# neggles/neurosis

Hardware: AMD Instinct MI355X
Metric: train images/sec (node) SDXL 1024^2 (higher is better)
Workload: dtype bf16

## Files before the change

include/neurosis_hip.h:

```cpp
#ifndef NEUROSIS_HIP_H
#define NEUROSIS_HIP_H

#ifdef __cplusplus
extern "C" {
#endif

const char* nk_last_error(void);
int nk_abi_version(void);

int nk_linear_fwd(const void* x, const void* w, const float* bias, const void* residual, void* y,
                  int M, int N, int K, long ldx, long ldw, long ldr, long ldy, float alpha, void* stream);
int nk_linear_dgrad(const void* dy, const void* w, const void* dx_add, void* dx, int M, int N, int K,
                    long lddy, long ldw, long ldadd, long lddx, void* stream);
long nk_linear_fwd_geglu_ok(int M, int I, int K);
int nk_linear_fwd_geglu(const void* x, const void* w, const float* bias, void* u, void* h, int M, int I, int K, long ldx, long ldw, long ldu,
                        long ldh, void* stream);
int nk_linear_dgrad_geglu(const void* dy, const void* w, const void* u, void* du, int M, int N, int I, long lddy, long ldw, long ldu,
                          long lddu, void* stream);
int nk_linear_fwd_geglu_s(const void* x, const void* w, const float* bias, void* s, void* h, int M, int I, int K, long ldx, long ldw, long lds,
                          long ldh, void* stream);
int nk_linear_dgrad_geglu_s(const void* dy, const void* w, const void* s, void* du, int M, int N, int I, long lddy, long ldw, long lds,
                            long lddu, void* stream);
int nk_linear_wgrad(const void* dy, const void* x, float* dw, int M, int N, int K, long lddy, long ldx,
                    long lddw, int accumulate, void* stream);
int nk_linear_wgrad_bias(const void* dy, const void* x, float* dw, float* dbias, int M, int N, int K, long lddy, long ldx, long lddw,
                         int accumulate, void* stream);

int nk_gemm_sk_status(void);

int nk_health_status(void);
int nk_health_clear(void);
int nk_health_export(int* dst, void* stream);
int nk_health_import(const int* src, void* stream);
int nk_debug_raise_health(void* stream);
int nk_debug_stamp(unsigned long long* dst, void* stream);
int nk_debug_launch_log(int mode);
long nk_debug_launch_names(char* buf, long cap);

int nk_colsum_batched(const void* dy, float* out, float* ws, long M, int N, long ld, int nbatch, int accumulate, void* stream);

int nk_linear_fwd_batched(const void* const* x, const void* const* w, void* const* y, int count, int M, int N, int K,
                          long ldx, long ldw, long ldy, void* stream);

int nk_linear_wgrad_batched(const void* const* dy, const void* const* x, float* const* dw, float* const* dbias, int count, int M, int N,
                            int K, long lddy, long ldx, long lddw, int accumulate, void* stream);

typedef struct NkConvDesc {
  int N, H, W, Cin;
  int Cout, KH, KW;
  int stride;
  int pad_t, pad_l;
  int Ho, Wo;
  int upsample;
} NkConvDesc;
int nk_conv2d_fwd(const NkConvDesc* d, const void* x, const void* w, const float* bias, const void* rowvec,
                  const void* residual, void* y, void* stream);
long nk_conv2d_stats_tiles(const NkConvDesc* d, int stats_groups);
int nk_conv2d_fwd_stats(const NkConvDesc* d, const void* x, const void* w, const float* bias, const void* rowvec, const void* residual,
                        void* y, float* stats_part, int stats_groups, void* stream);
int nk_conv3x3_few_channels_fwd(const void* x, const void* w, const float* bias, void* y, int N, int H, int W, int Cout, int cin_real,
                                void* stream);
int nk_conv_weight_flip(const void* w, void* wt, int Cout, int Cin, int taps, void* stream);
long nk_conv2d_dgrad_flipped_ok(const NkConvDesc* d);
int nk_conv2d_dgrad_flipped(const NkConvDesc* d, const void* dy, const void* wt, void* dx, void* stream);
int nk_conv2d_dgrad(const NkConvDesc* d, const void* dy, const void* w, void* dx, void* stream);
int nk_conv2d_wgrad(const NkConvDesc* d, const void* dy, const void* x, float* dw, int accumulate, void* stream);
int nk_conv2d_wgrad_bias(const NkConvDesc* d, const void* dy, const void* x, float* dw, float* dbias, int accumulate, void* stream);

typedef struct NkAttnDesc {
  int B, H, Lq, Lk, D;
  long sq, sk, sv, so;
  long bq, bk, bv, bo;
  long sdq, sdk, sdv, sdo;
  long bdq, bdk, bdv, bdo;
  float scale;
  int causal;
} NkAttnDesc;
int nk_attention_fwd(const NkAttnDesc* d, const void* q, const void* k, const void* v, void* o, float* lse,
                     void* stream);
long nk_attention_bwd_ws_floats(const NkAttnDesc* d);
int nk_attention_bwd(const NkAttnDesc* d, const void* q, const void* k, const void* v, const void* o,
// ... 166 lines not shown
```

neurosis_amd/csrc/conv_halo.h:

```cpp
#pragma once
#include <type_traits>

#ifdef NK_HALO_STAMPS
__device__ unsigned long long nk_halo_stamp_buf[8 * 8192];
__device__ unsigned long long nk_halo_kstep_buf[3 * 16 * 20 * 5];
#define CH_KSTAMP(t, ph) do { const int w_ = tid >> 6; if ((tid & 63) == 0 && (w_ == 0 || w_ == 4 || w_ == 6) && blockIdx.x >= 2048 && blockIdx.x < 2048 + 16 && (t) < 20) \
    nk_halo_kstep_buf[((((w_ == 0 ? 0 : (w_ == 4 ? 1 : 2)) * 16 + (blockIdx.x - 2048)) * 20 + (t)) * 5) + (ph)] = __builtin_amdgcn_s_memtime(); } while (0)
extern "C" int nk_debug_halo_ksteps(unsigned long long* host_out) {
  return hipMemcpyFromSymbol(host_out, HIP_SYMBOL(nk_halo_kstep_buf), sizeof(nk_halo_kstep_buf)) == hipSuccess ? 0 : 1;
}
#define CH_STAMP(slot) do { if (tid == 0 && blockIdx.x < 8192) nk_halo_stamp_buf[blockIdx.x * 8 + (slot)] = __builtin_amdgcn_s_memtime(); } while (0)
#define CH_STAMP_RT(slot) do { if (tid == 0 && blockIdx.x < 8192) nk_halo_stamp_buf[blockIdx.x * 8 + (slot)] = __builtin_amdgcn_s_memrealtime(); } while (0)
extern "C" int nk_debug_halo_stamps(unsigned long long* host_out, int nwg) {
  return hipMemcpyFromSymbol(host_out, HIP_SYMBOL(nk_halo_stamp_buf), (size_t)nwg * 8 * sizeof(unsigned long long)) == hipSuccess ? 0 : 1;
}
#else
#define CH_STAMP(slot)
#define CH_STAMP_RT(slot)
#define CH_KSTAMP(t, ph)
#endif
template <int BN_> struct HaloRing {
  static constexpr bool DEEP = BN_ == 128;
  static constexpr int BST = DEEP ? CH_BSTAGE_DEEP : CH_BSTAGE;
  static constexpr int NS = DEEP ? CH_NS_DEEP : CH_NS;
  static constexpr int AHEAD = 2;
  static constexpr bool PROD = BN_ == 128;
  static constexpr int THREADS = PROD ? 768 : 512;
  static constexpr int WAVES_PER_SIMD = PROD ? 3 : 2;
};
#define CH_NPROD_W 3
#define CH_NBW 6

template <int MI>
struct HaloGeom {
  static constexpr int TH = 2 * MI;
  static constexpr int RPW = MI / 2;
  static constexpr int HPX = (TH + 2) * CH_HW;
  static constexpr int HPIECES = ((HPX + 7) / 8 + 1) & ~1;
  static constexpr int HBUF = HPIECES * 1024;
  static constexpr int HPW = HPIECES / 2;
  static constexpr int SMEM = 2 * HBUF + CH_NS * CH_BSTAGE;
  static constexpr int SMEM_DEEP = 2 * HBUF + CH_NS_DEEP * CH_BSTAGE_DEEP;
  template <int BN_> static constexpr int smem() { return HaloRing<BN_>::DEEP ? SMEM_DEEP : SMEM; }
  static_assert(HPIECES == halo_hpieces(TH) && smem<128>() == halo_smem(128, TH) && smem<160>() == halo_smem(160, TH), "the planner's LDS size");
};
static_assert(HaloRing<128>::THREADS == halo_threads(128) && HaloRing<160>::THREADS == halo_threads(160), "the planner's block size");
constexpr int ch_count(int NPH, int LAST, int t) { return t > LAST ? 0 : (NPH + LAST - t) / (LAST + 1); }
constexpr int ch_start(int NPH, int LAST, int t) { int s = 0; for (int u = 0; u < t; ++u) s += ch_count(NPH, LAST, u); return s; }

template <int BN_, int NBW = CH_NBW>
struct HaloWeights {
  static constexpr int NPC = BN_ / 8;
  static constexpr int NPW = (NPC + NBW - 1) / NBW;
  const bf16_t* rp[NPW];
  bool ok[NPW];
  __device__ __forceinline__ static int pieces(int wave) { return wave >= NBW ? 0 : (wave + NBW * (NPW - 1) < NPC ? NPW : NPW - 1); }
  __device__ __forceinline__ void init(const bf16_t* Wt, long ld, int Cout, int n0, int wave, int lane) {
#pragma unroll
    for (int i = 0; i < NPW; ++i) {
      const int pc = wave + NBW * i;
      const int row = pc * 8 + (lane >> 3);
      const int chunk = (lane & 7) ^ (lane >> 3);
      ok[i] = wave < NBW && pc < NPC && n0 + row < Cout;
      rp[i] = Wt + (long)(n0 + (ok[i] ? row : 0)) * ld + chunk * 8;
    }
  }
  __device__ __forceinline__ void fire_next(bool live, long adv, char* img, int wave) {
    const bf16_t* zp = (const bf16_t*)nk_zero_page;
#pragma unroll
    for (int i = 0; i < NPW; ++i) {
      if (wave + NBW * i < NPC)
        __builtin_amdgcn_global_load_lds((nk_gptr)((live && ok[i]) ? rp[i] : zp), (nk_lptr)(img + (wave + NBW * i) * 1024), 16, 0, 0);
      rp[i] += adv;
    }
  }
};

template <int BN_, int MI, int STATS>
__global__ __launch_bounds__(HaloRing<BN_>::THREADS, HaloRing<BN_>::WAVES_PER_SIMD) void nk_conv3x3_halo_kernel(const NkGemmParams p) {
  extern __shared__ __attribute__((aligned(16))) char smem[];
  using G = HaloGeom<MI>;
  using R = HaloRing<BN_>;
  constexpr int HN = BN_ / 2, NJ = HN / 16;
  constexpr int RPW = G::RPW, HPW = G::HPW, HBUF = G::HBUF;
  constexpr int HLAST = 6;
  const int tid = threadIdx.x, lane = tid & 63;
  const int wave = __builtin_amdgcn_readfirstlane(tid >> 6);
  const int grp = wave >> 2, wq = wave & 3;
  constexpr bool PROD = HaloRing<BN_>::PROD;
  const bool hwave = !PROD && wave >= CH_NBW;
  CH_STAMP(0);

  const int H = p.ga.H, W = p.ga.W, Cin = p.ga.C, Cout = p.N;
  const int txn = (W + CH_TW - 1) / CH_TW, tyn = (H + G::TH - 1) / G::TH;
  const int per_img = txn * tyn;
  const int ntm = p.halo_nb * per_img, ntn = (Cout + BN_ - 1) / BN_;
  const int nwg = gridDim.x, bid = blockIdx.x;
  const int q8 = nwg >> 3, r8 = nwg & 7, xcd = bid & 7;
  const int wg = (xcd < r8 ? xcd * (q8 + 1) : r8 * (q8 + 1) + (xcd - r8) * q8) + (bid >> 3);
  constexpr int GM = 16;
  const int per_group = GM * ntn;
  const int group = wg / per_group;
  const int first_m = group * GM;
  const int gm = min(GM, ntm - first_m);
  const int in_group = wg - group * per_group;
  const int nt = in_group / gm;
  const int mt = first_m + (in_group - nt * gm);
  const int n0 = nt * BN_;
  const int img = mt / per_img;
  const int trem = mt - img * per_img;
  const int tyi = trem / txn;
  const int y0 = tyi * G::TH, x0 = (trem - tyi * txn) * CH_TW;
  const int nslab = Cin >> 6, nk = nslab * 9;

  typedef __attribute__((address_space(3))) const char* lds_c;
  const unsigned lds0 = (unsigned)(size_t)(lds_c)smem;
  char* const ring = smem + 2 * HBUF;

  constexpr int HPP = PROD ? G::HPIECES : HPW;
  const int hw = PROD ? 0 : wave - CH_NBW;
  const int hp0 = hw * HPP * 8 + (lane >> 3);
  auto fire_halo = [&](int i, int slab, char* hbuf) {
    const int hp = hp0 + 8 * i;
    const int py = hp / CH_HW, px = hp - py * CH_HW;
    const int y = y0 - 1 + py, x = x0 - 1 + px;
    const bool v = hp < G::HPX && (unsigned)y < (unsigned)H && (unsigned)x < (unsigned)W;
    const int chunk = (lane & 7) ^ (hp & 7);
    const bf16_t* src = v ? p.A + ((long)((img * H + y) * W + x) * Cin + chunk * 8 + slab * 64) : (const bf16_t*)nk_zero_page;
    __builtin_amdgcn_global_load_lds((nk_gptr)src, (nk_lptr)(hbuf + (hw * HPP + i) * 1024), 16, 0, 0);
  };

  using WB = HaloWeights<BN_, PROD ? CH_NPROD_W : CH_NBW>;
  const int sw = PROD ? wave - 8 : wave;
  WB wb;
  if (!PROD || wave >= 8) wb.init(p.B, p.ldb, Cout, n0, sw, lane);
  const long adv_tap = Cin, adv_slab = 64 - 8l * Cin;
  const int s0 = p.k_rotate ? (xcd * nslab) >> 3 : 0;
  const long adv_wrap = 64 - 9l * Cin;
#define CH_BAR() __builtin_amdgcn_sched_barrier(0); __builtin_amdgcn_s_barrier(); __builtin_amdgcn_sched_barrier(0)
  if constexpr (PROD) {
    if (wave >= 8) {
      const int pw = wave - 8;
      const bool halo_wave = pw == CH_NPROD_W;
      const int npw = WB::pieces(pw);
      if (halo_wave) {
#pragma unroll
        for (int i = 0; i < HPP; ++i) fire_halo(i, s0, smem);
        asm volatile("s_waitcnt vmcnt(0)" ::: "memory");
      } else {
#pragma unroll
        for (int i = 0; i < WB::NPW; ++i) wb.rp[i] += s0 * 64;
        wb.fire_next(true, adv_tap, ring, pw);
        wb.fire_next(nk > 1, adv_tap, ring + R::BST, pw);
        if (npw == 6) asm volatile("s_waitcnt vmcnt(6)" ::: "memory");
        else asm volatile("s_waitcnt vmcnt(5)" ::: "memory");
      }
      CH_BAR();
      unsigned sn = R::AHEAD * R::BST;
      int t = 0, sl = s0;
      for (int s = 0; s < nslab; ++s) {
        char* const hnext = smem + ((s + 1) & 1) * HBUF;
        const bool more = s + 1 < nslab;
        const int sln = sl + 1 == nslab ? 0 : sl + 1;
        const long adv_end = sl + 1 == nslab ? adv_wrap : adv_slab;
        auto pstep = [&](auto tapc) {
          constexpr int tap = decltype(tapc)::value;
          constexpr int tap2 = (tap + 2) % 9;
          if (!halo_wave) wb.fire_next(t + 2 < nk, tap2 == 8 ? adv_end : adv_tap, ring + sn, pw);
          CH_BAR();
          if (halo_wave) {
            if (more) {
              constexpr int cnt = ch_count(HPP, HLAST, tap), st = ch_start(HPP, HLAST, tap);
#pragma unroll
              for (int i = 0; i < cnt; ++i) fire_halo(st + i, sln, hnext);
            }
            if (tap == 8) asm volatile("s_waitcnt vmcnt(0)" ::: "memory");
          } else {
            if (npw == 6) asm volatile("s_waitcnt vmcnt(6)" ::: "memory");
            else asm volatile("s_waitcnt vmcnt(5)" ::: "memory");
          }
          CH_BAR();
          sn += R::BST; if (sn == R::NS * R::BST) sn = 0;
          ++t;
        };
        pstep(std::integral_constant<int, 0>{}); pstep(std::integral_constant<int, 1>{}); pstep(std::integral_constant<int, 2>{});
        pstep(std::integral_constant<int, 3>{}); pstep(std::integral_constant<int, 4>{}); pstep(std::integral_constant<int, 5>{});
        pstep(std::integral_constant<int, 6>{}); pstep(std::integral_constant<int, 7>{}); pstep(std::integral_constant<int, 8>{});
        sl = sln;
      }
      asm volatile("s_waitcnt vmcnt(0)" ::: "memory");
      CH_BAR();
      return;
    }
  } else {
#pragma unroll
    for (int i = 0; i < WB::NPW; ++i) wb.rp[i] += s0 * 64;
    if (hwave) {
#pragma unroll
      for (int i = 0; i < HPW; ++i) fire_halo(i, s0, smem);
    } else {
      wb.fire_next(true, adv_tap, ring, wave);
      wb.fire_next(nk > 1, adv_tap, ring + R::BST, wave);
    }
  }

  FragG2<OP_KC, BN_, NJ> fb;
  fb.init(lds0 + 2 * HBUF, grp * HN, lane);
  const int hpl = wq * RPW * CH_HW + (lane & 15);
  const int cl4 = lane >> 4;
  const int g4 = lane >> 4;
  const int nb = n0 + grp * HN;
  float4_t acc[MI][NJ];
#pragma unroll
  for (int i = 0; i < MI; ++i)
#pragma unroll
    for (int j = 0; j < NJ; ++j) acc[i][j] = (float4_t){0.f, 0.f, 0.f, 0.f};
  bf16x8_t af[2 * MI], bfr[2 * NJ];

  const int nbw = PROD ? 0 : WB::pieces(wave);

  if constexpr (!PROD) {
    if (hwave) {
      asm volatile("s_waitcnt vmcnt(0)" ::: "memory");
    } else {
      if (nbw == 4) asm volatile("s_waitcnt vmcnt(4)" ::: "memory");
      else if (nbw == 3) asm volatile("s_waitcnt vmcnt(3)" ::: "memory");
      else asm volatile("s_waitcnt vmcnt(2)" ::: "memory");
    }
  }
  CH_BAR();
  CH_STAMP(1); CH_STAMP_RT(4);
  if (grp == 1) { CH_BAR(); }

  unsigned so = 0, sn = R::AHEAD * R::BST;
  int t = 0;
  int sl = s0;
  for (int s = 0; s < nslab; ++s) {
    const unsigned hcur = lds0 + (unsigned)(s & 1) * HBUF;
    char* const hnext = smem + ((s + 1) & 1) * HBUF;
    const bool more = s + 1 < nslab;
    const int sln = sl + 1 == nslab ? 0 : sl + 1;
    const long adv_end = sl + 1 == nslab ? adv_wrap : adv_slab;
    auto step = [&](auto tapc) {
      constexpr int tap = decltype(tapc)::value;
      constexpr int dy = tap / 3, dx = tap % 3;
      __builtin_amdgcn_sched_barrier(0);
      int hpv = hpl;
      asm volatile("" : "+v"(hpv));
      g2_read<OP_KC, BN_, NJ>(bfr, fb, so);
#pragma unroll
      for (int r = 0; r < RPW; ++r) {
        const int hp = hpv + (r + dy) * CH_HW + dx;
        const unsigned ar = (unsigned)(hp * 128 + ((cl4 ^ (hp & 7)) << 4));
        const unsigned a0 = hcur + ar, a1 = hcur + (ar ^ 64u);
        G2_RD128(af[2 * r], a0, 0);
        G2_RD128(af[2 * r + 1], a0, 2048);
        G2_RD128(af[MI + 2 * r], a1, 0);
        G2_RD128(af[MI + 2 * r + 1], a1, 2048);
      }
      if constexpr (PROD) {
      } else if (hwave) {
        if (more) {
          constexpr int cnt = ch_count(HPW, HLAST, tap), st = ch_start(HPW, HLAST, tap);
#pragma unroll
          for (int i = 0; i < cnt; ++i) fire_halo(st + i, sln, hnext);
        }
        if (tap == 8) asm volatile("s_waitcnt vmcnt(0)" ::: "memory");
      } else {
        asm volatile("s_waitcnt vmcnt(0)" ::: "memory");
      }
      CH_KSTAMP(t, 4);
      CH_BAR();
      CH_KSTAMP(t, 0);
      asm volatile("s_waitcnt lgkmcnt(0)" ::: "memory");
      __builtin_amdgcn_sched_barrier(0);
      __builtin_amdgcn_s_setprio(1);
      if constexpr (!PROD) {
        if (!hwave) {
          constexpr int tap2 = (tap + 2) % 9;
          wb.fire_next(t + 2 < nk, tap2 == 8 ? adv_end : adv_tap, ring + sn, wave);
        }
      }
      CH_KSTAMP(t, 1);
#pragma unroll
      for (int ks = 0; ks < 2; ++ks)
#pragma unroll
        for (int i = 0; i < MI; ++i)
#pragma unroll
          for (int j = 0; j < NJ; ++j)
            acc[i][j] = __builtin_amdgcn_mfma_f32_16x16x32_bf16(bfr[ks * NJ + j], af[ks * MI + i], acc[i][j], 0, 0, 0);
      __builtin_amdgcn_s_setprio(0);
      CH_KSTAMP(t, 2);
      CH_BAR();
      CH_KSTAMP(t, 3);
      so += R::BST; if (so == R::NS * R::BST) so = 0;
      sn += R::BST; if (sn == R::NS * R::BST) sn = 0;
      ++t;
    };
    step(std::integral_constant<int, 0>{}); step(std::integral_constant<int, 1>{}); step(std::integral_constant<int, 2>{});
    step(std::integral_constant<int, 3>{}); step(std::integral_constant<int, 4>{}); step(std::integral_constant<int, 5>{});
    step(std::integral_constant<int, 6>{}); step(std::integral_constant<int, 7>{}); step(std::integral_constant<int, 8>{});
    sl = sln;
  }
  if (grp == 0) { CH_BAR(); }
  asm volatile("s_waitcnt vmcnt(0)" ::: "memory");
  CH_STAMP(2); CH_STAMP_RT(5);

  int mrow[MI];
  bool mok[MI];
#pragma unroll
  for (int i = 0; i < MI; ++i) {
    const int y = y0 + wq * RPW + (i >> 1), x = x0 + (i & 1) * 16 + (lane & 15);
    mok[i] = y < H && x < W;
    mrow[i] = (img * H + y) * W + x;
  }
  bf16_t* const C = (bf16_t*)p.C;
  uint4_t res8[MI][NJ / 2 ? NJ / 2 : 1];
  uint2_t res4[MI];
  if (p.residual) {
#pragma unroll
    for (int i = 0; i < MI; ++i) {
#pragma unroll
      for (int h = 0; h < NJ / 2; ++h) {
        const int n = nb + h * 32 + (g4 & 1) * 16 + (g4 >> 1) * 8;
        res8[i][h] = (mok[i] && n < Cout) ? *(const uint4_t*)(p.residual + (long)mrow[i] * p.ldr + n) : (uint4_t){0u, 0u, 0u, 0u};
      }
      if constexpr (NJ & 1) {
        const int n = nb + (NJ - 1) * 16 + g4 * 4;
        res4[i] = (mok[i] && n < Cout) ? *(const uint2_t*)(p.residual + (long)mrow[i] * p.ldr + n) : (uint2_t){0u, 0u};
      }
    }
  }
  float cadd[NJ / 2][8], cadd4[4];
#pragma unroll
  for (int h = 0; h < NJ / 2; ++h) {
    const int n = nb + h * 32 + (g4 & 1) * 16 + (g4 >> 1) * 8;
#pragma unroll
    for (int e = 0; e < 8; ++e) cadd[h][e] = 0.f;
    if (n < Cout) {
      if (p.bias) {
        const float4_t b0 = *(const float4_t*)(p.bias + n), b1 = *(const float4_t*)(p.bias + n + 4);
        cadd[h][0] = b0[0]; cadd[h][1] = b0[1]; cadd[h][2] = b0[2]; cadd[h][3] = b0[3];
        cadd[h][4] = b1[0]; cadd[h][5] = b1[1]; cadd[h][6] = b1[2]; cadd[h][7] = b1[3];
      }
      if (p.rowvec) {
        float t[8];
        unpack8(*(const uint4_t*)(p.rowvec + (long)img * p.ld_rowvec + n), t);
#pragma unroll
        for (int e = 0; e < 8; ++e) cadd[h][e] += t[e];
      }
    }
  }
#pragma unroll
  for (int e = 0; e < 4; ++e) cadd4[e] = 0.f;
  if constexpr (NJ & 1) {
    const int n = nb + (NJ - 1) * 16 + g4 * 4;
    if (n < Cout) {
// ... 123 lines not shown
```

neurosis_amd/csrc/gemm.hip:

```cpp
#include "nk_common.h"
#include "nk_gemm.h"
#include "gemm_plan.h"

#define NTHREADS 256
#define KC_IMAGE_BYTES (128 * 128)
#define MC_ROW_BYTES (128 * 2 + 16)
#define MC_IMAGE_BYTES (BK * MC_ROW_BYTES)
#define OPND_BYTES MC_IMAGE_BYTES
#define STAGE_BYTES (2 * OPND_BYTES)
#define SMEM_BYTES (2 * STAGE_BYTES)

static_assert(SMEM_BYTES >= BM * CS_LD * 4, "epilogue staging must fit");

__device__ __forceinline__ bool is_kc(int mode) { return mode == OP_KC || mode == OP_KCG; }

__device__ __forceinline__ long gather_offset(const NkGather& g, int n, int bh, int bw, int kh, int kw,
                                              int c, bool& valid) {
  int hn = bh + kh * g.ks;
  int wn = bw + kw * g.ks;
  bool ok = (hn >= 0) & (wn >= 0);
  ok &= (((hn | wn) & g.need_even) == 0);
  const int sh = g.div >> 1;
  int h = hn >> sh, w = wn >> sh;
  ok &= (h < g.H) & (w < g.W);
// ... 1335 lines not shown
        }
      const int mb = m0 + wm * 128 + ib * 64;
      if (p.geglu_save) {
        reg_epilogue_64x32<0>(ps, p.C, pa, mb, abase, lane);
        reg_epilogue_64x32<0>(ps, p.C, pg, mb, I + abase, lane);
      } else {
        reg_epilogue_64x32<0>(p, p.C, pa, mb, abase, lane);
        reg_epilogue_64x32<0>(p, p.C, pg, mb, I + abase, lane);
      }
      reg_epilogue_64x32<0>(ph, p.geglu_h, phh, mb, abase, lane);
    }
    return;
  }
#pragma unroll
  for (int ib = 0; ib < 2; ++ib)
#pragma unroll
    for (int half = 0; half < 2; ++half) {
      float4_t pair[4][2];
#pragma unroll
      for (int i = 0; i < 4; ++i) { pair[i][0] = acc[ib * 4 + i][2 * half]; pair[i][1] = acc[ib * 4 + i][2 * half + 1]; }
      reg_epilogue_64x32<0>(p, p.C, pair, m0 + wm * 128 + ib * 64, n0 + wn * 64 + half * 32, lane);
    }
}

__global__ void nk_zero_f32_kernel(float* __restrict__ dst, size_t n);
#include "gemm_g2.h"
#include "gemm_w160.h"
#include "conv_halo.h"
#include "conv_wgrad_halo.h"

typedef void (*NkGemmKernel)(const NkGemmParams);
static int launch_plan(NkGemmKernel kern, const NkGemmPlan& pl, const NkGemmParams& p, hipStream_t stream) {
  nk_optin_lds((const void*)kern, pl.smem);
  hipLaunchKernelGGL(kern, dim3(pl.grid[0], pl.grid[1], pl.grid[2]), dim3(pl.block), pl.smem, stream, p);
  return nk_check_launch(pl.name);
}

template <int A_, int B_, int F32_> struct Modes { static constexpr int A = A_, B = B_, F32 = F32_; };
template <class Fn>
static int with_modes(int amode, int bmode, int out_f32, Fn f) {
#define NK_CASE(A_, B_) \
  if (amode == A_ && bmode == B_) return out_f32 ? f(Modes<A_, B_, 1>()) : f(Modes<A_, B_, 0>());
  NK_CASE(OP_KC, OP_KC)
  NK_CASE(OP_KC, OP_MC)
  NK_CASE(OP_MC, OP_MC)
  NK_CASE(OP_KCG, OP_KC)
  NK_CASE(OP_KCG, OP_MCT)
  NK_CASE(OP_MC, OP_MCG)
#undef NK_CASE
  nk_set_error(__FILE__, __LINE__, "unsupported operand mode combination");
  return NK_ERR_ARG;
}

static NkGemmKernel halo_kernel(const NkGemmPlan& pl) {
  if (pl.bn == 160) {
    if (pl.halo_rows == 8) return pl.flag ? nk_conv3x3_halo_kernel<160, 4, 1> : nk_conv3x3_halo_kernel<160, 4, 0>;
    return pl.flag ? nk_conv3x3_halo_kernel<160, 2, 1> : nk_conv3x3_halo_kernel<160, 2, 0>;
  }
  if (pl.halo_rows == 8) return pl.flag ? nk_conv3x3_halo_kernel<128, 4, 1> : nk_conv3x3_halo_kernel<128, 4, 0>;
  return pl.flag ? nk_conv3x3_halo_kernel<128, 2, 1> : nk_conv3x3_halo_kernel<128, 2, 0>;
}

#include <mutex>
#include <unordered_map>
struct SkWorkspace {
  unsigned* flags = nullptr;
  float* ws = nullptr;
};
static std::mutex sk_mutex;
static std::unordered_map<void*, SkWorkspace> sk_spaces;

static int sk_prepare(NkGemmParams& p, hipStream_t stream) {
  std::lock_guard<std::mutex> lock(sk_mutex);
  SkWorkspace& w = sk_spaces[(void*)stream];
  if (!w.ws) {
    hipStreamCaptureStatus capturing = hipStreamCaptureStatusNone;
    if (hipStreamIsCapturing(stream, &capturing) == hipSuccess && capturing != hipStreamCaptureStatusNone) {
      nk_set_error(__FILE__, __LINE__, "stream-K workspace requested while the stream is capturing: run the launch once on this stream before capturing it");
      return NK_ERR_LAUNCH;
    }
    char* raw = nullptr;
    const size_t ws_bytes = (size_t)SK_MAX_GRID * SK_TILE_FLOATS * sizeof(float);
    if (hipMalloc((void**)&raw, ws_bytes + (SK_MAX_GRID + 64) * sizeof(unsigned)) != hipSuccess) {
      nk_set_error(__FILE__, __LINE__, "hipMalloc of the stream-K workspace failed");
      return NK_ERR_LAUNCH;
    }
    w.ws = (float*)raw;
    w.flags = (unsigned*)(raw + ws_bytes);
    if (hipMemsetAsync(w.flags, 0, (SK_MAX_GRID + 64) * sizeof(unsigned), stream) != hipSuccess) return NK_ERR_LAUNCH;
  }
  p.sk_health = nk_health_word();
  if (!p.sk_health) { nk_set_error(__FILE__, __LINE__, "health word allocation failed"); return NK_ERR_LAUNCH; }
  p.sk_flags = w.flags;
  p.sk_ws = w.ws;
  return NK_OK;
}

int nk_gemm_sk_reset(void) {
  std::lock_guard<std::mutex> lock(sk_mutex);
  for (auto& kv : sk_spaces)
    if (kv.second.flags && hipMemset(kv.second.flags, 0, (SK_MAX_GRID + 64) * sizeof(unsigned)) != hipSuccess) return NK_ERR_LAUNCH;
  return NK_OK;
}

extern "C" int nk_gemm_sk_status(void) {
  std::lock_guard<std::mutex> lock(sk_mutex);
  if (hipDeviceSynchronize() != hipSuccess) return -1;
  int bad = 0;
  for (auto& kv : sk_spaces) {
    unsigned v = 0;
    if (kv.second.flags && hipMemcpy(&v, kv.second.flags + SK_MAX_GRID + 1, sizeof(v), hipMemcpyDeviceToHost) == hipSuccess && v) bad = 1;
  }
  return bad;
}
// ... 16 lines not shown
  }
  return hipGetLastError() != hipSuccess ? NK_ERR_LAUNCH : NK_OK;
}

int nk_gemm_dispatch(NkGemmParams& p, int amode, int bmode, int out_f32, int allow_splitk,
                     hipStream_t stream) {
  NK_CHECK_ARG(p.M > 0 && p.N > 0 && p.K > 0);
  if (!p.nbatch) NK_CHECK_ARG(((uintptr_t)p.A & 15) == 0 && ((uintptr_t)p.B & 15) == 0 && ((uintptr_t)p.C & 15) == 0);
  for (int z = 0; z < p.nbatch; ++z) NK_CHECK_ARG(((uintptr_t)p.Ab[z] & 15) == 0 && ((uintptr_t)p.Bb[z] & 15) == 0 && ((uintptr_t)p.Cb[z] & 15) == 0);
  if (amode == OP_KC) NK_CHECK_ARG((p.K & 7) == 0 && (p.lda & 7) == 0);
  if (bmode == OP_KC) NK_CHECK_ARG((p.K & 7) == 0 && (p.ldb & 7) == 0);
  if (amode == OP_KCG) NK_CHECK_ARG((p.ga.C & 7) == 0);
  if (amode == OP_MC) NK_CHECK_ARG((p.M & 7) == 0 && (p.lda & 7) == 0);
  if (bmode == OP_MC) NK_CHECK_ARG((p.N & 7) == 0 && (p.ldb & 7) == 0);
  if (bmode == OP_MCT) NK_CHECK_ARG((p.N & 7) == 0 && (p.tw.co_stride & 7) == 0 && (p.tw.tap_stride & 7) == 0);
  if (bmode == OP_MCG) NK_CHECK_ARG((p.gb.C & 7) == 0);
  if (p.residual) NK_CHECK_ARG(((uintptr_t)p.residual & 15) == 0 && ((p.ldr & 7) == 0 || (p.N & 7) != 0));
  if (!out_f32) NK_CHECK_ARG((p.ldc & 7) == 0 || (p.N & 7) != 0);
  if (p.fRowsPerBatch.d == 0) p.fRowsPerBatch = make_fastdiv(1);

  if (p.dbias || (p.nbatch && p.dbias_b[0])) NK_CHECK_ARG(amode == OP_MC && out_f32);
  if (p.geglu_h) {
    NK_CHECK_ARG(amode == OP_KC && bmode == OP_KC && !out_f32 && !p.nbatch && (p.N & 255) == 0 && (p.ld_h & 7) == 0 && !p.rowvec && !p.residual && p.alpha == 1.0f);
    NK_CHECK_ARG(((uintptr_t)p.geglu_h & 15) == 0 && (!p.bias || ((uintptr_t)p.bias & 15) == 0));
  } else if (p.geglu_u) {
    NK_CHECK_ARG(amode == OP_KC && bmode == OP_MC && !out_f32 && !p.nbatch && (p.N & 7) == 0 && (p.ld_u & 7) == 0 && !p.bias && !p.rowvec && !p.residual);
  }

  const TileEnv env = tile_env();
  const NkGemmPlan pl = nk_gemm_plan(p, amode, bmode, out_f32, allow_splitk, env);
  if (pl.err) {
    nk_set_error(__FILE__, __LINE__, pl.err);
    return NK_ERR_ARG;
  }
  if (pl.zero_c) NK_CHECK_ARG(p.ldc == p.N);
  const int logging = nk_launch_log_mode();
  char line[192];
  if (logging) nk_plan_line(pl, line, sizeof(line));
  if (logging == 3) {
    nk_launch_log_add(pl.name, line);
    return NK_OK;
  }

  p.ksplit_len = pl.ksplit_len; p.accumulate = pl.accumulate; p.k_rotate = pl.k_rotate; p.group_m = pl.group_m; p.sk_chunked = pl.sk_chunked;
  if (pl.zero_c)
    if (int rc = zero_split_outputs(p, stream)) return rc;
  if (pl.family == NK_FAM_SK) {
    p.sk_debug = env.sk_debug;
    if (int rc = sk_prepare(p, stream)) return rc;
  }

  int rc;
  switch (pl.family) {
    case NK_FAM_HALO: rc = launch_plan(halo_kernel(pl), pl, p, stream); break;
    case NK_FAM_WGRAD_HALO: rc = launch_plan(pl.flag ? nk_conv3x3_wgrad_halo_kernel<1> : nk_conv3x3_wgrad_halo_kernel<0>, pl, p, stream); break;
    case NK_FAM_W160: rc = launch_plan(pl.bn == 160 ? nk_gemm_w160_kernel<160> : nk_gemm_w160_kernel<128>, pl, p, stream); break;
    case NK_FAM_RING64: rc = launch_plan(nk_gemm_ring64_kernel, pl, p, stream); break;
    case NK_FAM_XL: rc = launch_plan(nk_gemm_xl_kernel<OP_KCG, 64, 64>, pl, p, stream); break;
    case NK_FAM_XL2G: rc = launch_plan(pl.flag ? nk_gemm_xl2g_kernel<OP_KC, 1> : nk_gemm_xl2g_kernel<OP_KC, 0>, pl, p, stream); break;
    case NK_FAM_G2P:
      rc = with_modes(amode, bmode, out_f32, [&](auto m) {
        using M = decltype(m);
        if constexpr (M::B == OP_MCG) return (int)NK_ERR_ARG;
        else return launch_plan(pl.bn == 160 ? nk_gemm_g2p_kernel<M::A, M::B, M::F32, 160> : nk_gemm_g2p_kernel<M::A, M::B, M::F32, 128>, pl, p, stream);
      });
      break;
    case NK_FAM_SK:
      rc = with_modes(amode, bmode, out_f32, [&](auto m) { using M = decltype(m); return launch_plan(nk_gemm_sk_kernel<M::A, M::B, M::F32>, pl, p, stream); });
      break;
    case NK_FAM_RING:
      rc = with_modes(amode, bmode, out_f32, [&](auto m) { using M = decltype(m); return launch_plan(nk_gemm_ring_kernel<M::A, M::B, M::F32>, pl, p, stream); });
      break;
    case NK_FAM_DMA:
      rc = with_modes(amode, bmode, out_f32, [&](auto m) { using M = decltype(m); return launch_plan(nk_gemm_dma_kernel<M::A, M::B, M::F32, 8>, pl, p, stream); });
      break;
    default:
      nk_set_error(__FILE__, __LINE__, "the plan names no kernel");
      return NK_ERR_ARG;
  }
  if (logging) nk_launch_log_add(nullptr, line);
  return rc;
}

int nk_halo_tiles_per_image(const NkGemmParams& p, int* bn) {
  const NkGemmPlan pl = nk_gemm_plan(p, OP_KCG, OP_KC, 0, 0, tile_env());
  if (pl.err || pl.family != NK_FAM_HALO) return 0;
  if (bn) *bn = pl.bn;
  return pl.tiles_per_image;
}

int nk_geglu_fwd_fusable(const NkGemmParams& p) {
  if (p.N & 255) return 0;
  const NkGemmPlan pl = nk_gemm_plan(p, OP_KC, OP_KC, 0, 0, tile_env());
  return !pl.err && pl.family == NK_FAM_XL2G && pl.flag ? 1 : 0;
}
```

neurosis_amd/csrc/gemm_plan.h:

```cpp
#pragma once
#include "nk_gemm.h"
#include <stdio.h>
#include <stdlib.h>

enum { OP_KC = 0, OP_KCG = 1, OP_MC = 2, OP_MCT = 3, OP_MCG = 4 };

#define BM 128
#define BN 128
#define BK 64
#define GROUP_M 8
#define CS_LD 132
#define V2_OPND_BYTES 16384
#define V2_STAGE_BYTES (2 * V2_OPND_BYTES)
#define V2_SMEM_BYTES (BM * CS_LD * 4)
#define RING_NS 4
#define RING_SMEM_BYTES (RING_NS * V2_STAGE_BYTES)
#define SK_NT 512
#define SK_SMEM_BYTES (2 * V2_STAGE_BYTES)
#define SK_MAX_GRID 512
#define R64_NS 8
#define R64_OPND 8192
#define R64_STAGE (2 * R64_OPND)
#define R64_SMEM (R64_NS * R64_STAGE)
#define XL_BM 256
#define XL_BN 256
#define XL_STAGE_BYTES 65536
#define XL_SMEM_BYTES (2 * XL_STAGE_BYTES)
#define G2_BM 128
#define G2_STAGE_BYTES 36864
#define G2_NS 4
#define G2_SMEM_BYTES (G2_NS * G2_STAGE_BYTES)
#define W160_BM 160
#define W160_NS 3
constexpr int w160_smem(int bn) { return W160_NS * (W160_BM + bn) * 128; }
#define CH_TW 32
#define CH_HW (CH_TW + 2)
#define CH_BSTAGE 20480
#define CH_NS 3
#define CH_BSTAGE_DEEP 16384
#define CH_NS_DEEP 4
constexpr int halo_threads(int bn) { return bn == 128 ? 768 : 512; }
constexpr int halo_hpieces(int th) { return ((((th + 2) * CH_HW + 7) / 8) + 1) & ~1; }
constexpr int halo_smem(int bn, int th) { return 2 * halo_hpieces(th) * 1024 + (bn == 128 ? CH_NS_DEEP * CH_BSTAGE_DEEP : CH_NS * CH_BSTAGE); }
#define WH_TH 4
#define WH_TW 32
#define WH_HS 48
#define WH_X_BYTES ((WH_TH + 2) * WH_HS * 128)
#define WH_DY_BYTES (WH_TH * WH_TW * 256)
#define WH_STAGE (WH_X_BYTES + WH_DY_BYTES)
#define WH_SMEM (2 * WH_STAGE)
#define WH_BCO 128
#define WH_BCI 64

struct TileEnv {
  int xl;
  int g2;
  int sk;
  int sk_debug;
  int w160;
  int w160_split;
  int krot;
  int r64;
  int halo;
  int wgrad_halo;
};
static int env_int(const char* e, int unset) { return e ? atoi(e) : unset; }
static int env_not0(const char* e) { return !(e && e[0] == '0'); }
static TileEnv tile_env() {
  static const int xl = env_not0(getenv("NK_GEMM_XL"));
  TileEnv t;
  t.xl = xl;
  t.g2 = env_int(getenv("NK_GEMM_G2"), 1);
  t.sk = env_int(getenv("NK_GEMM_SK"), 4);
  t.sk_debug = env_int(getenv("NK_SK_DEBUG"), 0) & 2;
  t.w160 = env_int(getenv("NK_GEMM_W160"), 1);
  t.w160_split = env_int(getenv("NK_GEMM_W160_SPLIT"), 1);
  t.krot = env_int(getenv("NK_GEMM_KROT"), 1) != 0;
  t.r64 = env_not0(getenv("NK_GEMM_R64"));
  t.halo = env_not0(getenv("NK_CONV_HALO"));
  t.wgrad_halo = env_int(getenv("NK_CONV_WGRAD_HALO"), 1);
  return t;
}

enum NkFamily { NK_FAM_NONE = 0, NK_FAM_RING64, NK_FAM_G2P, NK_FAM_XL, NK_FAM_XL2G, NK_FAM_SK, NK_FAM_RING, NK_FAM_DMA, NK_FAM_W160, NK_FAM_HALO, NK_FAM_WGRAD_HALO };
struct NkGemmPlan {
  int family;
  int bn;
  int halo_rows;
  int flag;
  const char* name;
  unsigned grid[3];
  int block, smem;
  int splitk;
  int ksplit_len, accumulate, k_rotate, group_m, sk_chunked;
  bool zero_c, zero_dbias;
  int tiles_per_image;
  const char* err;
};

static void nk_plan_line(const NkGemmPlan& pl, char* buf, size_t cap) {
  snprintf(buf, cap, "%s grid=%u,%u,%u %d %d %d %d %d %d %d %d %d", pl.name, pl.grid[0], pl.grid[1], pl.grid[2], pl.block, pl.smem, pl.splitk,
           pl.ksplit_len, pl.accumulate, (pl.zero_c ? 1 : 0) | (pl.zero_dbias ? 2 : 0), pl.k_rotate, pl.group_m, pl.sk_chunked);
}

static int cdiv(long a, long b) { return (int)((a + b - 1) / b); }
static int nbatch1(const NkGemmParams& p) { return p.nbatch ? p.nbatch : 1; }
static bool has_dbias(const NkGemmParams& p) {
  bool any = p.dbias != nullptr;
  for (int z = 0; z < p.nbatch && z < NK_MAX_BATCH; ++z) any = any || p.dbias_b[z] != nullptr;
  return any;
}

static bool k_rotate_on(const TileEnv& env, int k_len) { return env.krot && (k_len + BK - 1) / BK >= 8; }

static bool use_xl(const TileEnv& env, const NkGemmParams& p, int amode, int bmode, int out_f32, int splitk) {
  if (!env.xl || p.nbatch || out_f32 || splitk != 1 || bmode != OP_KC || !(amode == OP_KC || amode == OP_KCG)) return false;
  const long ntn = (p.N + XL_BN - 1) / XL_BN;
  const long tiles = (long)((p.M + XL_BM - 1) / XL_BM) * ntn;
  const long rounds = (tiles + 255) / 256;
  return tiles >= 224 && tiles * 10 >= rounds * 256 * 8 && ntn * XL_BN * 100 <= (long)p.N * 112 && p.K >= 4 * BK;
}

static bool halo_shape_ok(const NkGemmParams& p) {
  const NkGather& g = p.ga;
  if (!p.halo_nb || g.KW != 3 || p.K != 9 * g.C || g.rs != 1 || g.ks != 1 || g.div != 1 || g.off_h != -1 || g.off_w != -1) return false;
  if (g.Ho != g.H || g.Wo != g.W || (g.C & 63) || p.alpha != 1.0f || p.nbatch) return false;
  if (p.N % 160 && p.N % 128) return false;
  if ((p.N & 7) || (p.ldc & 7) || (p.residual && (p.ldr & 7))) return false;
  return true;
}
static int halo_bn(int N) { return N % 160 == 0 ? 160 : 128; }
static int halo_tile_rows(const NkGemmParams& p) {
  const NkGather& g = p.ga;
// ... 284 lines not shown
```

neurosis_amd/lib.py:

```python
from __future__ import annotations

import ctypes as C
import os
from pathlib import Path

import torch

CSRC = Path(__file__).resolve().parent / "csrc"
LIB_PATH = CSRC / "libneurosis_hip.so"

vp, i32, i64, f32 = C.c_void_p, C.c_int, C.c_long, C.c_float


class NkConvDesc(C.Structure):
    _fields_ = [(n, i32) for n in ("N", "H", "W", "Cin", "Cout", "KH", "KW", "stride", "pad_t", "pad_l", "Ho", "Wo", "upsample")]


class NkAttnDesc(C.Structure):
    _fields_ = (
        [(n, i32) for n in ("B", "H", "Lq", "Lk", "D")]
        + [(n, i64) for n in ("sq", "sk", "sv", "so", "bq", "bk", "bv", "bo", "sdq", "sdk", "sdv", "sdo", "bdq", "bdk", "bdv", "bdo")]
        + [("scale", f32), ("causal", i32)]
    )

# ... 63 lines not shown
    "nk_lpips_layer_bwd": [vp, vp, vp, vp, vp, i32, i32, i32, f32, vp],
    "nk_batchnorm_fwd": [vp, vp, vp, vp, vp, vp, vp, vp, vp, i64, i32, f32, f32, f32, vp],
    "nk_batchnorm_bwd": [vp, vp, vp, vp, vp, vp, vp, vp, vp, vp, i64, i32, f32, i32, vp],
    "nk_batchnorm_eval": [vp, vp, vp, vp, vp, vp, vp, i64, i32, f32, f32, vp],
    "nk_silu_bwd": [vp, vp, vp, i64, vp],
    "nk_add": [vp, vp, vp, i64, vp],
    "nk_dropout": [vp, vp, vp, i64, i32, i64, i64, i64, vp, i32, i32, f32, vp],
    "nk_dropout_draw": [vp, vp, vp],
    "nk_cat_channels": [vp, vp, vp, i64, i32, i32, vp],
    "nk_split_channels": [vp, vp, vp, i64, i32, i32, vp],
    "nk_upsample2x_bwd": [vp, vp, i32, i32, i32, i32, vp],
    "nk_nchw_to_nhwc": [vp, i32, vp, i32, i32, i32, i32, f32, vp],
    "nk_nhwc_to_nchw": [vp, vp, i32, i32, i32, i32, i32, vp],
    "nk_cast_f32_to_bf16": [vp, vp, i64, vp],
    "nk_cast_bf16_to_f32": [vp, vp, i64, vp],
    "nk_colsum": [vp, vp, vp, i64, i32, i64, i32, vp],
    "nk_colsum_batched": [vp, vp, vp, i64, i32, i64, i32, i32, vp],
    "nk_timestep_embedding": [vp, vp, i32, i32, f32, vp],
    "nk_edm_prepare": [vp, vp, vp, vp, vp, vp, i32, i32, i32, i32, vp],
    "nk_edm_loss": [vp, vp, vp, vp, vp, vp, vp, vp, i32, i32, i32, i32, f32, vp],
    "nk_sample_prepare": [vp, vp, vp, i32, i32, i32, i32, i32, vp],
    "nk_sample_denoise": [vp, vp, vp, vp, f32, vp, i32, i32, i32, i32, i32, vp],
    "nk_sample_euler_step": [vp, vp, vp, vp, vp, vp, f32, vp, vp, i32, i32, i32, i32, i32, vp],
    "nk_adamw_flat": [vp, vp, vp, vp, vp, i64, f32, f32, f32, f32, f32, i32, f32, vp],
    "nk_ema_flat": [vp, vp, i64, f32, vp],
    "nk_debug_raise_health": [vp],
    "nk_debug_stamp": [vp, vp],
    "nk_debug_launch_log": [i32],
    "nk_health_clear": [],
    "nk_health_export": [vp, vp],
    "nk_health_import": [vp, vp],
    "nk_adafactor_init": [vp, vp],
    "nk_adafactor_chunk": [vp, vp],
    "nk_came_chunk": [vp, vp],
    "nk_adamw8bit_step": [vp, vp],
}

SIZE_QUERIES: dict[str, list] = {
    "nk_groupnorm_ws_floats": [i32, i32, i32, i32],
    "nk_groupnorm_sums_ws_floats": [i32, i32, i32],
    "nk_conv2d_stats_tiles": [cdp, i32],
    "nk_conv2d_dgrad_flipped_ok": [cdp],
    "nk_linear_fwd_geglu_ok": [i32, i32, i32],
    "nk_layernorm_ws_floats": [i32, i32],
    "nk_layernorm_part_rows": [i32],
    "nk_colsum_ws_floats": [i64, i32],
    "nk_batchnorm_ws_floats": [i64, i32],
    "nk_lpips_layer_ws_floats": [i32, i32],
    "nk_attention_bwd_ws_floats": [adp],
    "nk_adafactor_tensor_bytes": [],
    "nk_came_tensor_bytes": [],
    "nk_adamw8bit_tensor_bytes": [],
    "nk_gemm_sk_status": [],
    "nk_health_status": [],
    "nk_debug_launch_names": [C.c_char_p, i64],
}

_lib = None


class NkError(RuntimeError):
    pass


def load() -> C.CDLL:
    global _lib
    if _lib is not None:
        return _lib
    path = Path(os.environ.get("NEUROSIS_HIP_LIB", LIB_PATH))
    if not path.exists():
        raise NkError(
            f"{path} not found: the HIP extension is not built. Run `python -c 'import __graft_entry__ as g; g.build()'` "
            "(or `make -C neurosis_amd/csrc`). There is no CPU fallback for the product path."
        )
    lib = C.CDLL(str(path))
    lib.nk_last_error.restype = C.c_char_p
    lib.nk_last_error.argtypes = []
    lib.nk_abi_version.restype = i32
    lib.nk_abi_version.argtypes = []
    for name, argtypes in SIGNATURES.items():
        fn = getattr(lib, name)
        fn.argtypes = argtypes
        fn.restype = i32
    for name, argtypes in SIZE_QUERIES.items():
        fn = getattr(lib, name)
        fn.argtypes = argtypes
        fn.restype = i64
    _lib = lib
    return lib


def launch_log(mode: int) -> None:
    call("nk_debug_launch_log", int(mode))


def launched() -> list[str]:
    buf = C.create_string_buffer(8192)
    n = query("nk_debug_launch_names", buf, len(buf))
    if n < 0:
        raise NkError("nk_debug_launch_names failed")
    return buf.value.decode().split("\n")[:-1]


def query(name: str, *args) -> int:
    return int(getattr(load(), name)(*args))

# ... 7 lines not shown
```

Measured before the change: 26.36.

## Add self-pipelined halo conv main loop with register double-buffered LDS reads

Adds a LOOP=1 variant of the 3x3 halo conv kernel for the 128-column tile. Each consumer wave double-buffers its B and A fragments in registers and interleaves the next k-substep's LDS reads between MFMAs, using counted lgkmcnt waits and sched barriers. Producer waves get a matching simplified fire/wait schedule, and the two-group barrier stagger is replaced by a single per-step barrier. The variant is on by default through NK_CONV_HALO_LOOP; it costs extra registers and depends on hand-counted waits being correct.

```diff
diff --git a/include/neurosis_hip.h b/include/neurosis_hip.h
--- a/include/neurosis_hip.h
+++ b/include/neurosis_hip.h
@@ -27,6 +27,8 @@
                          int accumulate, void* stream);
 
 int nk_gemm_sk_status(void);
+
+int nk_conv_halo_loop(void);
 
 int nk_health_status(void);
 int nk_health_clear(void);
diff --git a/neurosis_amd/csrc/conv_halo.h b/neurosis_amd/csrc/conv_halo.h
--- a/neurosis_amd/csrc/conv_halo.h
+++ b/neurosis_amd/csrc/conv_halo.h
@@ -4,7 +4,7 @@
 #ifdef NK_HALO_STAMPS
 __device__ unsigned long long nk_halo_stamp_buf[8 * 8192];
 __device__ unsigned long long nk_halo_kstep_buf[3 * 16 * 20 * 5];
-#define CH_KSTAMP(t, ph) do { const int w_ = tid >> 6; if ((tid & 63) == 0 && (w_ == 0 || w_ == 4 || w_ == 6) && blockIdx.x >= 2048 && blockIdx.x < 2048 + 16 && (t) < 20) \
+#define CH_KSTAMP(t, ph) do { const int w_ = tid >> 6; if ((tid & 63) == 0 && (w_ == 0 || w_ == 4 || w_ == KSW) && blockIdx.x >= 2048 && blockIdx.x < 2048 + 16 && (t) < 20) \
     nk_halo_kstep_buf[((((w_ == 0 ? 0 : (w_ == 4 ? 1 : 2)) * 16 + (blockIdx.x - 2048)) * 20 + (t)) * 5) + (ph)] = __builtin_amdgcn_s_memtime(); } while (0)
 extern "C" int nk_debug_halo_ksteps(unsigned long long* host_out) {
   return hipMemcpyFromSymbol(host_out, HIP_SYMBOL(nk_halo_kstep_buf), sizeof(nk_halo_kstep_buf)) == hipSuccess ? 0 : 1;
@@ -76,8 +76,20 @@
   }
 };
 
-template <int BN_, int MI, int STATS>
+template <int FIRST, int LAST, class F>
+__device__ __forceinline__ void ch_for(F&& f) {
+  if constexpr (FIRST < LAST) { f(std::integral_constant<int, FIRST>{}); ch_for<FIRST + 1, LAST>(f); }
+}
+
+template <int R, int NJ, int MI>
+__device__ __forceinline__ void ch_issue_read(bf16x8_t (&bq)[NJ], bf16x8_t (&aq)[MI], unsigned bb, const unsigned (&aa)[MI / 2]) {
+  if constexpr (R < NJ) G2_RD128(bq[R], bb, R * 2048);
+  else G2_RD128(aq[R - NJ], aa[(R - NJ) >> 1], ((R - NJ) & 1) * 2048);
+}
+
+template <int BN_, int MI, int STATS, int LOOP = 0>
 __global__ __launch_bounds__(HaloRing<BN_>::THREADS, HaloRing<BN_>::WAVES_PER_SIMD) void nk_conv3x3_halo_kernel(const NkGemmParams p) {
+  static_assert(LOOP == 0 || HaloRing<BN_>::PROD, "the self-pipelined loop needs the producer waves");
   extern __shared__ __attribute__((aligned(16))) char smem[];
   using G = HaloGeom<MI>;
   using R = HaloRing<BN_>;
@@ -88,6 +100,7 @@
   const int wave = __builtin_amdgcn_readfirstlane(tid >> 6);
   const int grp = wave >> 2, wq = wave & 3;
   constexpr bool PROD = HaloRing<BN_>::PROD;
+  [[maybe_unused]] constexpr int KSW = LOOP == 1 ? 8 : 6;
   const bool hwave = !PROD && wave >= CH_NBW;
   CH_STAMP(0);
 
@@ -156,6 +169,45 @@
         else asm volatile("s_waitcnt vmcnt(5)" ::: "memory");
       }
       CH_BAR();
+      if constexpr (LOOP == 1) {
+        unsigned sn = R::AHEAD * R::BST;
+        int t = 0, sl = s0;
+        for (int s = 0; s < nslab; ++s) {
+          char* const hnext = smem + ((s + 1) & 1) * HBUF;
+          const bool more = s + 1 < nslab;
+          const int sln = sl + 1 == nslab ? 0 : sl + 1;
+          const long adv_end = sl + 1 == nslab ? adv_wrap : adv_slab;
+          auto pstep = [&](auto tapc) {
+            constexpr int tap = decltype(tapc)::value;
+            constexpr int tap2 = (tap + 2) % 9;
+            CH_KSTAMP(t, 0);
+            if (halo_wave) {
+              if (more) {
+                constexpr int cnt = ch_count(HPP, HLAST, tap), st = ch_start(HPP, HLAST, tap);
+#pragma unroll
+                for (int i = 0; i < cnt; ++i) fire_halo(st + i, sln, hnext);
+              }
+              if (tap == 8) asm volatile("s_waitcnt vmcnt(0)" ::: "memory");
+            } else {
+              wb.fire_next(t + 2 < nk, tap2 == 8 ? adv_end : adv_tap, ring + sn, pw);
+              CH_KSTAMP(t, 1);
+              if (npw == 6) asm volatile("s_waitcnt vmcnt(6)" ::: "memory");
+              else asm volatile("s_waitcnt vmcnt(5)" ::: "memory");
+            }
+            CH_KSTAMP(t, 2);
+            CH_BAR();
+            sn += R::BST; if (sn == R::NS * R::BST) sn = 0;
+            ++t;
+          };
+          pstep(std::integral_constant<int, 0>{}); pstep(std::integral_constant<int, 1>{}); pstep(std::integral_constant<int, 2>{});
+          pstep(std::integral_constant<int, 3>{}); pstep(std::integral_constant<int, 4>{}); pstep(std::integral_constant<int, 5>{});
+          pstep(std::integral_constant<int, 6>{}); pstep(std::integral_constant<int, 7>{}); pstep(std::integral_constant<int, 8>{});
+          sl = sln;
+        }
+        asm volatile("s_waitcnt vmcnt(0)" ::: "memory");
+        CH_BAR();
+        return;
+      }
       unsigned sn = R::AHEAD * R::BST;
       int t = 0, sl = s0;
       for (int s = 0; s < nslab; ++s) {
@@ -230,6 +282,94 @@
   }
   CH_BAR();
   CH_STAMP(1); CH_STAMP_RT(4);
+  if constexpr (LOOP == 1) {
+    constexpr int NRD = NJ + MI;
+    constexpr int GAPS = (MI - 1) * NJ;
+    static_assert(NJ == 4 && (MI == 2 || MI == 4), "the counted waits below are written for the 128-column tile");
+    bf16x8_t bq[2][NJ], aq[2][MI];
+    unsigned aa[RPW];
+    auto a_addr = [&](int hpv, int dy, int dx, unsigned hb, unsigned ks64) {
+#pragma unroll
+      for (int r = 0; r < RPW; ++r) {
+        const int hp = hpv + (r + dy) * CH_HW + dx;
+        aa[r] = hb + ((unsigned)(hp * 128 + ((cl4 ^ (hp & 7)) << 4)) ^ ks64);
+      }
+    };
+    auto substep = [&](auto ks_tag, int tt, unsigned bb) {
+      constexpr int KS = decltype(ks_tag)::value, NXT = 1 - KS;
+      if constexpr (KS == 1) {
+        if constexpr (MI == 4)
+          asm volatile("s_waitcnt lgkmcnt(0)" : "+v"(bq[1][0]), "+v"(bq[1][1]), "+v"(bq[1][2]), "+v"(bq[1][3]), "+v"(aq[1][0]), "+v"(aq[1][1]), "+v"(aq[1][2]), "+v"(aq[1][3]));
+        else
+          asm volatile("s_waitcnt lgkmcnt(0)" : "+v"(bq[1][0]), "+v"(bq[1][1]), "+v"(bq[1][2]), "+v"(bq[1][3]), "+v"(aq[1][0]), "+v"(aq[1][1]));
+      } else {
+        asm volatile("s_waitcnt lgkmcnt(%5)" : "+v"(bq[0][0]), "+v"(bq[0][1]), "+v"(bq[0][2]), "+v"(bq[0][3]), "+v"(aq[0][0]) : "n"(MI - 1));
+      }
+      __builtin_amdgcn_sched_barrier(0);
+#pragma unroll
+      for (int j = 0; j < NJ; ++j)
+        acc[0][j] = __builtin_amdgcn_mfma_f32_16x16x32_bf16(bq[KS][j], aq[KS][0], acc[0][j], 0, 0, 0);
+      if constexpr (KS == 1) {
+        CH_KSTAMP(tt, 3);
+        CH_BAR();
+        CH_KSTAMP(tt, 0);
+      }
+      __builtin_amdgcn_sched_barrier(0);
+      ch_for<1, MI>([&](auto i_tag) {
+        constexpr int i = decltype(i_tag)::value;
+        if constexpr (KS == 0) {
+          constexpr int allow = (MI - 1 - i) + ((i - 1) * NJ * NRD + GAPS - 1) / GAPS;
+          asm volatile("s_waitcnt lgkmcnt(%1)" : "+v"(aq[0][i]) : "n"(allow));
+          __builtin_amdgcn_sched_barrier(0);
+        }
+        ch_for<0, NJ>([&](auto j_tag) {
+          constexpr int j = decltype(j_tag)::value;
+          constexpr int g = (i - 1) * NJ + j;
+          constexpr int r0 = (g * NRD + GAPS - 1) / GAPS, r1 = ((g + 1) * NRD + GAPS - 1) / GAPS;
+          acc[i][j] = __builtin_amdgcn_mfma_f32_16x16x32_bf16(bq[KS][j], aq[KS][i], acc[i][j], 0, 0, 0);
+          ch_for<r0, r1>([&](auto r_tag) { ch_issue_read<decltype(r_tag)::value>(bq[NXT], aq[NXT], bb, aa); });
+          __builtin_amdgcn_sched_barrier(0);
+        });
+      });
+    };
+
+    a_addr(hpl, 0, 0, lds0, 0u);
+    ch_for<0, NRD>([&](auto r_tag) { ch_issue_read<decltype(r_tag)::value>(bq[0], aq[0], fb.a[0], aa); });
+    if constexpr (MI == 4)
+      asm volatile("s_waitcnt lgkmcnt(0)" : "+v"(bq[0][0]), "+v"(bq[0][1]), "+v"(bq[0][2]), "+v"(bq[0][3]), "+v"(aq[0][0]), "+v"(aq[0][1]), "+v"(aq[0][2]), "+v"(aq[0][3]));
+    else
+      asm volatile("s_waitcnt lgkmcnt(0)" : "+v"(bq[0][0]), "+v"(bq[0][1]), "+v"(bq[0][2]), "+v"(bq[0][3]), "+v"(aq[0][0]), "+v"(aq[0][1]));
+    __builtin_amdgcn_sched_barrier(0);
+    __builtin_amdgcn_s_setprio(1);
+    unsigned so = 0;
+    int t = 0;
+    for (int s = 0; s < nslab; ++s) {
+      const unsigned hcur = lds0 + (unsigned)(s & 1) * HBUF, hnx = lds0 + (unsigned)((s + 1) & 1) * HBUF;
+      auto step = [&](auto tapc) {
+        constexpr int tap = decltype(tapc)::value, tapn = (tap + 1) % 9;
+        int hpv = hpl;
+        asm volatile("" : "+v"(hpv));
+        unsigned son = so + R::BST; if (son == R::NS * R::BST) son = 0;
+        a_addr(hpv, tap / 3, tap % 3, hcur, 64u);
+        substep(std::integral_constant<int, 0>{}, t, fb.a[1] + so);
+        a_addr(hpv, tapn / 3, tapn % 3, tap == 8 ? hnx : hcur, 0u);
+        substep(std::integral_constant<int, 1>{}, t, fb.a[0] + son);
+        CH_KSTAMP(t, 2);
+        so = son;
+        ++t;
+      };
+      step(std::integral_constant<int, 0>{}); step(std::integral_constant<int, 1>{}); step(std::integral_constant<int, 2>{});
+      step(std::integral_constant<int, 3>{}); step(std::integral_constant<int, 4>{}); step(std::integral_constant<int, 5>{});
+      step(std::integral_constant<int, 6>{}); step(std::integral_constant<int, 7>{}); step(std::integral_constant<int, 8>{});
+    }
+    if constexpr (MI == 4)
+      asm volatile("s_waitcnt lgkmcnt(0)" : "+v"(bq[0][0]), "+v"(bq[0][1]), "+v"(bq[0][2]), "+v"(bq[0][3]), "+v"(aq[0][0]), "+v"(aq[0][1]), "+v"(aq[0][2]), "+v"(aq[0][3]));
+    else
+      asm volatile("s_waitcnt lgkmcnt(0)" : "+v"(bq[0][0]), "+v"(bq[0][1]), "+v"(bq[0][2]), "+v"(bq[0][3]), "+v"(aq[0][0]), "+v"(aq[0][1]));
+    __builtin_amdgcn_sched_barrier(0);
+    __builtin_amdgcn_s_setprio(0);
+    CH_BAR();
+  } else {
   if (grp == 1) { CH_BAR(); }
 
   unsigned so = 0, sn = R::AHEAD * R::BST;
@@ -303,6 +443,7 @@
     sl = sln;
   }
   if (grp == 0) { CH_BAR(); }
+  }
   asm volatile("s_waitcnt vmcnt(0)" ::: "memory");
   CH_STAMP(2); CH_STAMP_RT(5);
 
diff --git a/neurosis_amd/csrc/gemm.hip b/neurosis_amd/csrc/gemm.hip
--- a/neurosis_amd/csrc/gemm.hip
+++ b/neurosis_amd/csrc/gemm.hip
@@ -1411,14 +1411,19 @@
   return NK_ERR_ARG;
 }
 
-static NkGemmKernel halo_kernel(const NkGemmPlan& pl) {
+static NkGemmKernel halo_kernel(const NkGemmPlan& pl, const TileEnv& env) {
   if (pl.bn == 160) {
     if (pl.halo_rows == 8) return pl.flag ? nk_conv3x3_halo_kernel<160, 4, 1> : nk_conv3x3_halo_kernel<160, 4, 0>;
     return pl.flag ? nk_conv3x3_halo_kernel<160, 2, 1> : nk_conv3x3_halo_kernel<160, 2, 0>;
   }
+  if (env.halo_loop) {
+    if (pl.halo_rows == 8) return pl.flag ? nk_conv3x3_halo_kernel<128, 4, 1, 1> : nk_conv3x3_halo_kernel<128, 4, 0, 1>;
+    return pl.flag ? nk_conv3x3_halo_kernel<128, 2, 1, 1> : nk_conv3x3_halo_kernel<128, 2, 0, 1>;
+  }
   if (pl.halo_rows == 8) return pl.flag ? nk_conv3x3_halo_kernel<128, 4, 1> : nk_conv3x3_halo_kernel<128, 4, 0>;
   return pl.flag ? nk_conv3x3_halo_kernel<128, 2, 1> : nk_conv3x3_halo_kernel<128, 2, 0>;
 }
+extern "C" int nk_conv_halo_loop(void) { return tile_env().halo_loop; }
 
 #include <mutex>
 #include <unordered_map>
@@ -1541,7 +1546,7 @@
 
   int rc;
   switch (pl.family) {
-    case NK_FAM_HALO: rc = launch_plan(halo_kernel(pl), pl, p, stream); break;
+    case NK_FAM_HALO: rc = launch_plan(halo_kernel(pl, env), pl, p, stream); break;
     case NK_FAM_WGRAD_HALO: rc = launch_plan(pl.flag ? nk_conv3x3_wgrad_halo_kernel<1> : nk_conv3x3_wgrad_halo_kernel<0>, pl, p, stream); break;
     case NK_FAM_W160: rc = launch_plan(pl.bn == 160 ? nk_gemm_w160_kernel<160> : nk_gemm_w160_kernel<128>, pl, p, stream); break;
     case NK_FAM_RING64: rc = launch_plan(nk_gemm_ring64_kernel, pl, p, stream); break;
diff --git a/neurosis_amd/csrc/gemm_plan.h b/neurosis_amd/csrc/gemm_plan.h
--- a/neurosis_amd/csrc/gemm_plan.h
+++ b/neurosis_amd/csrc/gemm_plan.h
@@ -63,6 +63,7 @@
   int r64;
   int halo;
   int wgrad_halo;
+  int halo_loop;
 };
 static int env_int(const char* e, int unset) { return e ? atoi(e) : unset; }
 static int env_not0(const char* e) { return !(e && e[0] == '0'); }
@@ -79,6 +80,7 @@
   t.r64 = env_not0(getenv("NK_GEMM_R64"));
   t.halo = env_not0(getenv("NK_CONV_HALO"));
   t.wgrad_halo = env_int(getenv("NK_CONV_WGRAD_HALO"), 1);
+  t.halo_loop = env_not0(getenv("NK_CONV_HALO_LOOP"));
   return t;
 }
 
diff --git a/neurosis_amd/lib.py b/neurosis_amd/lib.py
--- a/neurosis_amd/lib.py
+++ b/neurosis_amd/lib.py
@@ -139,6 +139,7 @@
     "nk_came_tensor_bytes": [],
     "nk_adamw8bit_tensor_bytes": [],
     "nk_gemm_sk_status": [],
+    "nk_conv_halo_loop": [],
     "nk_health_status": [],
     "nk_debug_launch_names": [C.c_char_p, i64],
 }
```

After: 26.45 (median of 3 runs). About the same (+0.3%).
